# caesar-one/audio-classification-using-a-deep-cnn-combined-with-multi-level-attention

Measured on AMD Instinct MI355X. Metric: 0.96 s clips/sec wave->logits (VGGish+attn), higher is better.
Workload: dtype bf16; 1 GPU; BASELINE config 3: wave->logits forward, 1024 bags x 10 s 16 kHz PCM per GPU = 10240 x 0.96 s clips per step, VGGish + MLA [2,1], random-init portable-seeded weights; f32 front-end/head, bf16 conv+FC; bags_per_gpu=1024, parallelism=dp1 (no collective: independent bags)

## Files before the change

### audio-classification-using-a-deep-cnn-combined-with-multi-level-attention_amd/_lib.py

```python

import ctypes
import os
import re

HERE = os.path.dirname(os.path.abspath(__file__))
LIB_PATH = os.environ.get("MLA_HIP_LIB") or os.path.join(HERE, "libmla_hip.so")
HEADER = os.path.join(os.path.dirname(HERE), "include", "mla_hip.h")

F32, BF16, I16, BF16X3, F64, I32 = 0, 1, 2, 3, 4, 5
E_SHORT = -3

_lib = None


class MlaError(RuntimeError):
    def __init__(self, code, msg):
        super().__init__("libmla_hip error %d: %s" % (code, msg))
        self.code = code


def declared_symbols():
    text = open(HEADER).read()
    text = re.sub(r"/\*.*?\*/", "", text, flags=re.S)
    return sorted(set(re.findall(r"\b(mla_[a-z0-9_]+)\s*\(", text)))
# ... 3 lines not shown
    global _lib
    if _lib is None:
        if not os.path.exists(LIB_PATH):
            raise RuntimeError(
                "%s is missing: build it with `python __graft_entry__.py` (hipcc --offload-arch=gfx950). "
                "There is no fallback path." % LIB_PATH)
        import torch
        L = ctypes.CDLL(LIB_PATH)
        L.mla_last_error.restype = ctypes.c_char_p
        L.mla_logmel_table_floats.restype = ctypes.c_int64
        i64, vp, ci = ctypes.c_int64, ctypes.c_void_p, ctypes.c_int
        L.mla_logmel_counts.argtypes = [i64, ctypes.POINTER(i64), ctypes.POINTER(i64)]
        L.mla_logmel_build_tables.argtypes = [vp]
        L.mla_logmel_reference_tables.argtypes = [vp, vp]
        L.mla_logmel_examples.argtypes = [vp, ci, i64, i64, i64, vp, vp, ci, vp]
        cf = ctypes.c_float
        L.mla_stft_magnitude.argtypes = [vp, i64, vp, vp, i64, i64, i64, vp, vp]
        L.mla_mel_log.argtypes = [vp, vp, i64, i64, i64, cf, vp, vp]
        L.mla_dataset_frames.argtypes = [vp, i64, ci, ci, ci, ci, vp, vp]
        L.mla_postprocess.argtypes = [vp, vp, vp, i64, vp, vp]
        L.mla_mono_mix.argtypes = [vp, ci, i64, ci, vp, vp]
        L.mla_split_bf16x3.argtypes = [vp, i64, i64, i64, vp, i64, i64, ci, vp]
        L.mla_merge_bf16x3.argtypes = [vp, i64, i64, i64, i64, vp, vp]
        L.mla_linear_bf16x3.argtypes = [vp, i64, vp, i64, vp, vp, i64, i64, i64, i64, i64, ci, ci, vp]
        L.mla_conv_repack_weights.argtypes = [vp, i64, i64, vp, ci, vp]
        L.mla_convert_f32.argtypes = [vp, vp, i64, ci, vp]
        L.mla_convert_bf16_to_f32.argtypes = [vp, vp, i64, vp]
        L.mla_vggish_conv1.argtypes = [vp, ci, i64, vp, vp, vp, ci, vp]
        L.mla_vggish_conv.argtypes = [ci, vp, vp, vp, vp, i64, ci, vp]
        L.mla_linear.argtypes = [vp, i64, vp, i64, vp, vp, i64, i64, i64, i64, ci, ci, ci, vp]
# ... 97 lines not shown
```

### audio-classification-using-a-deep-cnn-combined-with-multi-level-attention_amd/csrc/conv.hip

```cpp
#include <cstdlib>
#include <type_traits>

#include "common.h"
#include "mma_core.h"

namespace {

using namespace mma;

constexpr int kThreads = 512, kWaves = 8, kMS = 6;

#ifndef MLA_CONV_STAMPS
#define MLA_CONV_STAMPS 0
#endif
#ifndef MLA_STAMP_TAP
#define MLA_STAMP_TAP 4
#define MLA_STAMP_CHUNK 5
#endif
#if MLA_CONV_STAMPS
__device__ unsigned long long g_conv_stamps[8][2][8];
#define MLA_STAMP(k) do { if (stamp_on) stamps[k] = __builtin_amdgcn_s_memtime(); } while (0)
#if MLA_CONV_STAMPS == 2
#undef MLA_STAMP
#define MLA_STAMP(k) do { } while (0)
// ... 604 lines not shown
    __builtin_amdgcn_wave_barrier();
    __builtin_amdgcn_fence(__ATOMIC_ACQUIRE, "wavefront");
    constexpr int PIECES = 64 * int(sizeof(T)) / 16;
    char* dst = reinterpret_cast<char*>(out + ((size_t(img) * 48 + y0 / 2 + wave) * 32) * 64);
    _Pragma("unroll") for (int it = 0; it < PIECES / 2; ++it) {
        const int piece = it * 64 + lane, p = piece / PIECES, c = piece % PIECES;
        *reinterpret_cast<u32x4*>(dst + size_t(piece) * 16) = *reinterpret_cast<const u32x4*>(stage + p * ROW + c * 16);
    }
    __syncthreads();
    }
}

template <typename TIN>
__global__ __launch_bounds__(256, MLA_CONV1_WAVES) void conv1_patch_kernel(const TIN* __restrict__ x, const float* __restrict__ w,
                                                            const float* __restrict__ bias, bf16_t* __restrict__ out, int n_img) {
    typedef float f32x16 __attribute__((ext_vector_type(16)));
    constexpr int TR = MLA_CONV1_ROWS;
    constexpr int TPC = 96 / TR;
    constexpr int NP = (TR + 2) * 66;
    constexpr int NL = (NP + 255) / 256;
    constexpr int PITCH = 68;
    constexpr int ROW = 64 * 2 + 16;
    __shared__ __attribute__((aligned(16))) uint16_t sX[(TR + 2) * PITCH];
    __shared__ __attribute__((aligned(16))) char sOut[4 * 32 * ROW];
    const int t = threadIdx.x, lane = t & 63, wave = t >> 6, px = lane & 31, h = lane >> 5;
    const int n_tiles = n_img * TPC;

    bf16x8 wa[4][2];
    f32x16 binit[2];
    {
        const int rho = px;
        const int chl = 16 * ((rho >> 2) & 1) + (rho & 3) + 4 * (rho >> 3);
        _Pragma("unroll") for (int pos = 0; pos < 4; ++pos) {
            const int dy = pos >> 1, dx = pos & 1;
            _Pragma("unroll") for (int mt = 0; mt < 2; ++mt) {
                const int ch = mt * 32 + chl;
                uint32_t pk[4];
                _Pragma("unroll") for (int jj = 0; jj < 4; ++jj) {
                    float v[2];
                    _Pragma("unroll") for (int e = 0; e < 2; ++e) {
                        const int k = 8 * h + 2 * jj + e, i = k >> 2, c = k & 3;
                        const int ky = i - dy, kx = c - dx;
                        v[e] = (ky >= 0 && ky < 3 && kx >= 0 && kx < 3) ? w[ch * 9 + ky * 3 + kx] : 0.f;
                    }
                    pk[jj] = pack_bf16x2(v[0], v[1]);
                }
                wa[pos][mt] = __builtin_bit_cast(bf16x8, u32x4{pk[0], pk[1], pk[2], pk[3]});
            }
        }
        _Pragma("unroll") for (int mt = 0; mt < 2; ++mt)
            _Pragma("unroll") for (int reg = 0; reg < 16; ++reg) binit[mt][reg] = bias[mt * 32 + 16 * h + reg];
    }

    float pre[NL];
    auto patch_load = [&](int tile) {
        const int img = tile / TPC, y0 = (tile % TPC) * TR;
        _Pragma("unroll") for (int k = 0; k < NL; ++k) {
            const int p = t + 256 * k, yh = p / 66, xh = p % 66;
            const int gy = y0 + yh - 1, gx = xh - 1;
            const int cy = gy < 0 ? 0 : (gy > 95 ? 95 : gy), cx = gx < 0 ? 0 : (gx > 63 ? 63 : gx);
            const float v = load_elem<TIN>(x + (size_t(img) * 96 + cy) * 64 + cx);
            pre[k] = (p < NP && gy >= 0 && gy < 96 && gx >= 0 && gx < 64) ? v : 0.f;
        }
    };
    auto patch_write = [&]() {
        _Pragma("unroll") for (int k = 0; k < NL; ++k) {
            const int p = t + 256 * k;
// ... 6 lines not shown
        __builtin_amdgcn_s_barrier();
#else
        __syncthreads();
#endif
    };
    int tile = blockIdx.x;
    if (tile < n_tiles) patch_load(tile);
    char* stage = sOut + wave * 32 * ROW;
    for (; tile < n_tiles; tile += gridDim.x) {
        const int img = tile / TPC, y0 = (tile % TPC) * TR;
        patch_write();
        lds_barrier();
        if (tile + int(gridDim.x) < n_tiles) patch_load(tile + int(gridDim.x));
        _Pragma("unroll") for (int rr = 0; rr < TR / 8; ++rr) {
            const int prow = wave * (TR / 8) + rr;
            const uint32_t* r0 = reinterpret_cast<const uint32_t*>(sX + (2 * prow + 2 * h) * PITCH) + px;
            const uint32_t* r1 = reinterpret_cast<const uint32_t*>(sX + (2 * prow + 2 * h + 1) * PITCH) + px;
            const bf16x8 bfrag = __builtin_bit_cast(bf16x8, u32x4{r0[0], r0[1], r1[0], r1[1]});
            _Pragma("unroll") for (int mt = 0; mt < 2; ++mt) {
                f32x16 m = __builtin_amdgcn_mfma_f32_32x32x16_bf16(wa[0][mt], bfrag, binit[mt], 0, 0, 0);
                _Pragma("unroll") for (int pos = 1; pos < 4; ++pos) {
                    const f32x16 a = __builtin_amdgcn_mfma_f32_32x32x16_bf16(wa[pos][mt], bfrag, binit[mt], 0, 0, 0);
                    _Pragma("unroll") for (int reg = 0; reg < 16; ++reg) m[reg] = fmaxf(m[reg], a[reg]);
                }
                uint32_t pk[8];
                _Pragma("unroll") for (int e = 0; e < 8; ++e) pk[e] = pack_bf16x2(fmaxf(m[2 * e], 0.f), fmaxf(m[2 * e + 1], 0.f));
                char* dst = stage + px * ROW + (mt * 32 + 16 * h) * 2;
                *reinterpret_cast<u32x4*>(dst) = u32x4{pk[0], pk[1], pk[2], pk[3]};
                *reinterpret_cast<u32x4*>(dst + 16) = u32x4{pk[4], pk[5], pk[6], pk[7]};
            }
            __builtin_amdgcn_fence(__ATOMIC_RELEASE, "wavefront");
            __builtin_amdgcn_wave_barrier();
            __builtin_amdgcn_fence(__ATOMIC_ACQUIRE, "wavefront");
            char* gdst = reinterpret_cast<char*>(out + ((size_t(img) * 48 + y0 / 2 + prow) * 32) * 64);
            _Pragma("unroll") for (int it = 0; it < 4; ++it) {
                const int piece = it * 64 + lane, p = piece >> 3, c = piece & 7;
#if MLA_CONV_NT_STORE
                __builtin_nontemporal_store(*reinterpret_cast<const u32x4*>(stage + p * ROW + c * 16), reinterpret_cast<u32x4*>(gdst + size_t(piece) * 16));
#else
                *reinterpret_cast<u32x4*>(gdst + size_t(piece) * 16) = *reinterpret_cast<const u32x4*>(stage + p * ROW + c * 16);
#endif
            }
            __builtin_amdgcn_fence(__ATOMIC_RELEASE, "wavefront");
            __builtin_amdgcn_wave_barrier();
            __builtin_amdgcn_fence(__ATOMIC_ACQUIRE, "wavefront");
        }
        lds_barrier();
    }
}

template <typename T>
__global__ void repack_kernel(const float* __restrict__ w, T* __restrict__ out, int cout, int cin) {
    const int64_t total = int64_t(cout) * 9 * cin;
    for (int64_t i = int64_t(blockIdx.x) * blockDim.x + threadIdx.x; i < total; i += int64_t(gridDim.x) * blockDim.x) {
        const int c = int(i % cin);
        const int tap = int((i / cin) % 9);
        const int o = int(i / (int64_t(cin) * 9));
        store_elem<T>(out + i, w[(int64_t(o) * cin + c) * 9 + tap]);
    }
}
// ... 325 lines not shown
```

### audio-classification-using-a-deep-cnn-combined-with-multi-level-attention_amd/csrc/logmel.hip

```cpp
#include <hip/hip_bf16.h>

#include "common.h"
#include "logmel_core.h"
#include "logmel_tables.h"

namespace {

using namespace logmel;

#ifndef MLA_LOGMEL_STAMPS
#define MLA_LOGMEL_STAMPS 0
#endif
#if MLA_LOGMEL_STAMPS
__device__ unsigned long long g_logmel_stamps[256][10];
#endif

constexpr int kPair = 2;
constexpr int kChunk = 16 * kPair;
constexpr int kThreads = 256;
constexpr int kWgPerCu = 2;
constexpr int kXchFloats = 2 * 16 * kXchStride;
constexpr int kWinFloats = 416;
constexpr int kPwPitch = 18;
constexpr int kU = 18;
// ... 102 lines not shown
        _Pragma("unroll") for (int e = 0; e < 4; ++e) {
            _Pragma("unroll") for (int s = 0; s < 4; ++s) {
                if (t < count[s]) {
                    acc_a[s] += w[first[s] / 4 + t][e] * a[first[s] / 4 + t][e];
                    acc_b[s] += w[first[s] / 4 + t][e] * b[first[s] / 4 + t][e];
                }
            }
        }
    }
    _Pragma("unroll") for (int s = 0; s < 4; ++s) {
        oa[s] = __builtin_amdgcn_logf(acc_a[s] + 0.01f) * 0.69314718055994530942f;
        ob[s] = __builtin_amdgcn_logf(acc_b[s] + 0.01f) * 0.69314718055994530942f;
    }
}

template <typename OutT>
__device__ __forceinline__ void store_piece(OutT* dst, f32x4 v) {
    if constexpr (sizeof(OutT) == 4) {
        *reinterpret_cast<f32x4*>(dst) = v;
    } else {
        const __hip_bfloat16 b0 = __float2bfloat16(v.x), b1 = __float2bfloat16(v.y), b2 = __float2bfloat16(v.z), b3 = __float2bfloat16(v.w);
        auto bits = [](const __hip_bfloat16& h) { return uint32_t(*reinterpret_cast<const uint16_t*>(&h)); };
        *reinterpret_cast<u32x2*>(dst) = u32x2{bits(b0) | (bits(b1) << 16), bits(b2) | (bits(b3) << 16)};
    }
}

template <typename InT, typename OutT, bool VEC, bool WAVE>
__device__ __forceinline__ void pair_step(const LaneConsts& c, int j, Samples<InT>& smp, const InT* next_frame, float* xa, float* xb,
                                          const float* s_win, const float* melw, const float* pw, OutT* dst) {
    float ra[16], ia[16], rb[16], ib[16];
    {
        _Pragma("unroll") for (int n1 = 0; n1 < kN1; ++n1) {
            const f32x2 w = *reinterpret_cast<const f32x2*>(s_win + 32 * n1 + 2 * j);
            const f32x2 a = smp.pair(n1), b = smp.pair(n1 + 5);
            ra[n1] = a.x * w.x; ia[n1] = a.y * w.y;
            rb[n1] = b.x * w.x; ib[n1] = b.y * w.y;
        }
    }
    if (next_frame) smp.template fetch<VEC>(next_frame, j);
    phase1_fft(c, j, ra, ia, xa);
    group_sync<WAVE>();
    phase1_fft(c, j, rb, ib, xb);
    group_sync<WAVE>();
    read_row(xa + 2 * (j * kXchStride), ra, ia);
// ... 5 lines not shown
    }
    __builtin_amdgcn_sched_barrier(0);
    group_sync<WAVE>();
    phase2_fft(ra, ia);
    split_frame<WAVE>(j, ra, ia, xa, pwl);
    phase2_fft(rb, ib);
    split_frame<WAVE>(j, rb, ib, xb, pwl);
    group_sync<WAVE>();
    float oa[4], ob[4];
    mel_pair(c, xa, xb, melw, oa, ob);
    _Pragma("unroll") for (int s = 0; s < 4; ++s) { xa[256 + band_of(j, s)] = oa[s]; xb[256 + band_of(j, s)] = ob[s]; }
    group_sync<WAVE>();
    {
        const f32x4 va = *reinterpret_cast<const f32x4*>(xa + 256 + 4 * j);
        const f32x4 vb = *reinterpret_cast<const f32x4*>(xb + 256 + 4 * j);
        store_piece<OutT>(dst + 4 * j, va);
        store_piece<OutT>(dst + kBands + 4 * j, vb);
    }
    group_sync<WAVE>();
}

template <typename InT, typename OutT, bool VEC, bool WAVE>
__global__ __launch_bounds__(kThreads, kWgPerCu) void logmel_kernel(const InT* __restrict__ pcm, ChunkMap map,
                                                              int64_t n_chunks, const float* __restrict__ tab,
                                                              OutT* __restrict__ out) {
    extern __shared__ __attribute__((aligned(16))) float smem[];
    float* s_xch = smem;
    float* s_mel = s_xch + kChunk * kXchFloats;
    float* s_pw = s_mel + 16 * kMelRow;
    float* s_win = s_pw + 16 * kPwPitch;

    const int t = threadIdx.x, g = t >> 4, j = t & 15;
// ... 12 lines not shown
    Samples<InT> smp;
    int64_t chunk = blockIdx.x, sample0, row0;
    if (chunk < n_chunks) {
        map.locate(chunk, sample0, row0);
        smp.template fetch<VEC>(pcm + sample0 + (kPair * g) * kHop, j);
    }
    for (; chunk < n_chunks; chunk += gridDim.x) {
        map.locate(chunk, sample0, row0);
        const int64_t next = chunk + gridDim.x;
        const InT* next_frame = nullptr;
        if (next < n_chunks) {
            int64_t ns, nr;
            map.locate(next, ns, nr);
            next_frame = pcm + ns + (kPair * g) * kHop;
        }
        pair_step<InT, OutT, VEC, WAVE>(c, j, smp, next_frame, xa, xb, s_win, melw, pw, out + (row0 + kPair * g) * kBands);
    }
}

constexpr int kThreadsDyn = 512;
constexpr int kItemFrames = 4 * kPair;
constexpr int kLdsFloatsDyn = (kThreadsDyn / 16) * kPair * kXchFloats + 16 * kMelRow + 16 * kPwPitch + kWinFloats + 4;
constexpr int kLdsBytesDyn = kLdsFloatsDyn * 4;
static_assert(kLdsBytesDyn <= 160 * 1024 && kChunk % kItemFrames == 0, "dynamic kernel: LDS / item size");

template <typename InT, typename OutT, bool VEC>
__global__ __launch_bounds__(kThreadsDyn, 1) void logmel_dyn_kernel(const InT* __restrict__ pcm, ChunkMap map, int64_t n_items,
                                                                    const float* __restrict__ tab, OutT* __restrict__ out) {
    extern __shared__ __attribute__((aligned(16))) float smem[];
    float* s_xch = smem;
    float* s_mel = s_xch + (kThreadsDyn / 16) * kPair * kXchFloats;
// ... 39 lines not shown
    if (cur < hi) {
        locate_item(cur, sample, row);
        smp.template fetch<VEC>(pcm + sample + lane_frame * kHop, j);
    }
#if MLA_LOGMEL_STAMPS
    const unsigned long long stamp0 = __builtin_amdgcn_s_memrealtime();
#endif
    while (cur < hi) {
        const int nxt = pull();
        int64_t nsample = 0, nrow = 0;
        const InT* next_frame = nullptr;
        if (nxt < hi) {
            locate_item(nxt, nsample, nrow);
            next_frame = pcm + nsample + lane_frame * kHop;
        }
        pair_step<InT, OutT, VEC, true>(c, j, smp, next_frame, xa, xb, s_win, melw, pw, out + (row + lane_frame) * kBands);
        cur = nxt;
        row = nrow;
    }
#if MLA_LOGMEL_STAMPS
    if (lane == 0 && blockIdx.x < 256) {
        if (t == 0) { g_logmel_stamps[blockIdx.x][0] = stamp_entry; g_logmel_stamps[blockIdx.x][9] = stamp0; }
        g_logmel_stamps[blockIdx.x][1 + (t >> 6)] = __builtin_amdgcn_s_memrealtime();
    }
#endif
}

template <typename InT, typename OutT>
int launch(const void* pcm, int64_t n_wave, int64_t wave_stride, int64_t examples, const float* tables,
           void* out, bool wave_sync, bool static_wave, hipStream_t stream) {
    const int64_t n_chunks = n_wave * examples * (kExFrames / kChunk);
    if (n_chunks == 0) return MLA_OK;
    const bool vec = mla::aligned(pcm, 2 * sizeof(InT)) && (wave_stride % 2 == 0);
    int dev = 0, cus = 256;
    if (hipGetDevice(&dev) == hipSuccess) hipDeviceGetAttribute(&cus, hipDeviceAttributeMultiprocessorCount, dev);
    const int64_t grid = n_chunks < kWgPerCu * int64_t(cus) ? n_chunks : kWgPerCu * int64_t(cus);
    ChunkMap map{wave_stride, int(examples * (kExFrames / kChunk))};
    auto go = [&](auto kern) -> int {
        MLA_HIP_OK(hipFuncSetAttribute(reinterpret_cast<const void*>(kern),
                                       hipFuncAttributeMaxDynamicSharedMemorySize, kLdsBytes));
// ... 70 lines not shown
    MLA_REQUIRE(pcm && tables && out, MLA_E_ARG, "null pcm/tables/out");
    MLA_REQUIRE(mla::aligned(out, 16) && mla::aligned(tables, 4), MLA_E_ARG, "out must be 16-byte aligned");
    MLA_REQUIRE(pcm_dtype == MLA_F32 || pcm_dtype == MLA_I16, MLA_E_DTYPE, "pcm_dtype %d", pcm_dtype);
    MLA_REQUIRE(out_dtype == MLA_F32 || out_dtype == MLA_BF16, MLA_E_DTYPE, "out_dtype %d", out_dtype);
    MLA_REQUIRE(mla::aligned(pcm, pcm_dtype == MLA_F32 ? 4 : 2), MLA_E_ARG, "pcm misaligned for its dtype");
    const char* env = getenv("MLA_LOGMEL_SYNC");
    const bool wave_sync = !(env && env[0] == 'b'), static_wave = env && env[0] == 's';
    hipStream_t s = static_cast<hipStream_t>(stream);
    if (pcm_dtype == MLA_F32) {
        return out_dtype == MLA_F32 ? launch<float, float>(pcm, n_wave, wave_stride, examples, tables, out, wave_sync, static_wave, s)
                                    : launch<float, __hip_bfloat16>(pcm, n_wave, wave_stride, examples, tables, out, wave_sync, static_wave, s);
    }
    return out_dtype == MLA_F32 ? launch<int16_t, float>(pcm, n_wave, wave_stride, examples, tables, out, wave_sync, static_wave, s)
                                : launch<int16_t, __hip_bfloat16>(pcm, n_wave, wave_stride, examples, tables, out, wave_sync, static_wave, s);
}
```

### audio-classification-using-a-deep-cnn-combined-with-multi-level-attention_amd/model.py

```python

from typing import Dict, List, Union

import torch
from torch import nn

from . import differentiable, mla_train, ops, resnet
from .params import *
from .torchvggish.vggish import Linear, VGGish


class BatchNorm1d(nn.Module):

    def __init__(self, num_features):
        super().__init__()
        self.num_features, self.eps, self.momentum = num_features, 1e-5, 0.1
        self.weight = nn.Parameter(torch.ones(num_features))
        self.bias = nn.Parameter(torch.zeros(num_features))
        self.register_buffer("running_mean", torch.zeros(num_features))
        self.register_buffer("running_var", torch.ones(num_features))
        self.register_buffer("num_batches_tracked", torch.tensor(0, dtype=torch.long))

    def forward(self, x):
        raise RuntimeError("BatchNorm1d is executed by the fused HIP head of its parent module")

# ... 56 lines not shown
    def forward(self, x):
        x_proc = self.input(x)
        features = self.cnn(x_proc)
        out = self.mla(features.reshape(-1, T, self.emb_input_size))
        return out

    def _waveforms_only_vggish(self):
        if self.cnn_type != "vggish":
            raise NotImplementedError("the waveform paths feed VGGish log-mel examples; cnn_type 'resnet' takes 224 x 224 "
                                      "spectrogram images (dataset.py:175-178 of the reference) through forward()")

    def forward_waveforms(self, pcm):
        self._waveforms_only_vggish()
        from . import frontend
        dtype = torch.bfloat16 if self.cnn.precision == "bf16" else torch.float32
        ex = frontend.waveforms_to_examples(pcm, out_dtype=dtype)
        assert ex.shape[0] == pcm.shape[0] * T, "each waveform must yield exactly T examples"
        features = self.cnn(ex)
        return self.mla(features.reshape(-1, T, self.emb_input_size))

    def stream_waveforms(self, host_batches):
        self._waveforms_only_vggish()
        dev = next(self.parameters()).device
        cur = torch.cuda.current_stream(dev)
        copy = torch.cuda.Stream(device=dev)
        it = iter(host_batches)

        def upload(host):
            assert host.is_pinned(), "stream_waveforms overlaps asynchronous copies: the host tensors must be pinned"
            with torch.cuda.stream(copy):
# ... 204 lines not shown
```

### audio-classification-using-a-deep-cnn-combined-with-multi-level-attention_amd/ops.py

```python

import ctypes

import torch

from . import _lib

DT = {torch.float32: _lib.F32, torch.bfloat16: _lib.BF16, torch.int16: _lib.I16}
BN_EPS = 1e-5

profile = None
_ws = {}


_event_pool = []


def reserve_events(n):
    while len(_event_pool) < n:
        e = torch.cuda.Event(enable_timing=True)
        e.record()
        _event_pool.append(e)
    torch.cuda.synchronize()


# ... 75 lines not shown

def to_f32(x):
    _chk(x, torch.bfloat16)
    out = torch.empty(x.shape, dtype=torch.float32, device=x.device)
    _lib.check(_lib.lib().mla_convert_bf16_to_f32(_p(x), _p(out), x.numel(), _lib.stream_ptr()))
    return out


def conv1(x, w, b, dtype, split=False):
    _chk(x); _chk(w, torch.float32); _chk(b, torch.float32)
    n = x.shape[0]
    assert tuple(x.shape[1:]) == (96, 64) and tuple(w.shape) == (64, 1, 3, 3)
    out = torch.empty((n, 48, 32, 128 if split else 64), dtype=dtype, device=x.device)
    _lib.check(_timed("conv1", _lib.lib().mla_vggish_conv1, _p(x), DT[x.dtype], n, _p(w), _p(b), _p(out),
                      _lib.BF16X3 if split else DT[dtype], _lib.stream_ptr()))
    return out


CONV_SHAPES = {2: ((48, 32, 64), (24, 16, 128)), 3: ((24, 16, 128), (24, 16, 256)), 4: ((24, 16, 256), (12, 8, 256)),
               5: ((12, 8, 256), (12, 8, 512)), 6: ((12, 8, 512), (6, 4, 512))}


def conv(layer, x, w_packed, b, split=False):
    _chk(x); _chk(w_packed, x.dtype); _chk(b, torch.float32)
    shp_in, shp_out = CONV_SHAPES[layer]
    ka, kw, ko = (2, 3, 2) if split else (1, 1, 1)
    assert tuple(x.shape[1:]) == shp_in[:2] + (ka * shp_in[2],), (x.shape, shp_in)
    assert tuple(w_packed.shape) == (shp_out[2], 9, kw * shp_in[2])
    n = x.shape[0]
    out = torch.empty((n,) + shp_out[:2] + (ko * shp_out[2],), dtype=x.dtype, device=x.device)
# ... 680 lines not shown
```

### audio-classification-using-a-deep-cnn-combined-with-multi-level-attention_amd/torchvggish/vggish.py

```python

import math

import numpy as np
import torch
import torch.nn as nn

from . import vggish_input, vggish_params
from .. import ops

_DTYPES = {"f32": torch.float32, "bf16": torch.bfloat16, "bf16x3": torch.bfloat16}


class Conv3x3(nn.Module):

    def __init__(self, in_channels, out_channels):
        super().__init__()
        self.in_channels, self.out_channels = in_channels, out_channels
        self.weight = nn.Parameter(torch.empty(out_channels, in_channels, 3, 3))
        self.bias = nn.Parameter(torch.empty(out_channels))
        nn.init.kaiming_uniform_(self.weight, a=math.sqrt(5))
        bound = 1.0 / math.sqrt(in_channels * 9)
        nn.init.uniform_(self.bias, -bound, bound)

    def forward(self, x):
# ... 13 lines not shown
    pass


class _Cache:

    def __init__(self):
        self.key, self.val = None, None

    def get(self, params, dtype, make):
        key = (dtype,) + tuple((p.data_ptr(), p._version) for p in params)
        if key != self.key:
            self.key, self.val = key, make()
        return self.val


class VGGFeatures(nn.Sequential):

    precision = "f32"

    def __init__(self, *layers):
        super().__init__(*layers)
        self._cache = _Cache()
        convs = [m for m in self if isinstance(m, Conv3x3)]
        assert [(c.in_channels, c.out_channels) for c in convs] == [(1, 64), (64, 128), (128, 256), (256, 256), (256, 512), (512, 512)]
        self._convs = convs

    def forward_nhwc(self, x, dtype):
        x = x.detach().reshape(-1, 96, 64)
        if x.dtype not in (torch.float32, torch.bfloat16):
            x = x.float()
        x = x.contiguous()
        convs = self._convs
        if self.precision == "bf16x3":
            packed = self._cache.get([c.weight for c in convs[1:]], "bf16x3",
                                     lambda: [ops.split_conv_weight(c.weight.detach().contiguous()) for c in convs[1:]])
            h = ops.conv1(x.float(), convs[0].weight.detach().contiguous(), convs[0].bias.detach(), torch.bfloat16, split=True)
            for layer, (c, w) in enumerate(zip(convs[1:], packed), start=2):
                h = ops.conv(layer, h, w, c.bias.detach(), split=True)
            return h
        packed = self._cache.get([c.weight for c in convs[1:]], dtype,
                                 lambda: [ops.repack_conv_weight(c.weight.detach().contiguous(), dtype) for c in convs[1:]])
        h = ops.conv1(x, convs[0].weight.detach().contiguous(), convs[0].bias.detach(), dtype)
        for layer, (c, w) in enumerate(zip(convs[1:], packed), start=2):
            h = ops.conv(layer, h, w, c.bias.detach())
        return h

    def forward(self, x):
        from .. import differentiable as D
        if D.wants_grad(self):
            params = [t for i in (0, 3, 6, 8, 11, 13) for t in (self[i].weight, self[i].bias)]
            return D.FeaturesFn.apply(self, D.grad_precision(self.precision), x, *params).permute(0, 3, 1, 2)
        return self.forward_nhwc(x, _DTYPES[self.precision]).permute(0, 3, 1, 2)


class Linear(nn.Module):

    def __init__(self, in_features, out_features):
        super().__init__()
        self.in_features, self.out_features = in_features, out_features
        self.weight = nn.Parameter(torch.empty(out_features, in_features))
        self.bias = nn.Parameter(torch.empty(out_features))
        nn.init.kaiming_uniform_(self.weight, a=math.sqrt(5))
        bound = 1.0 / math.sqrt(in_features)
# ... 134 lines not shown
```

### include/mla_hip.h

```cpp
#ifndef MLA_HIP_H
#define MLA_HIP_H

#include <stdint.h>

#ifdef __cplusplus
extern "C" {
#endif

#define MLA_OK            0
#define MLA_E_ARG        -1
#define MLA_E_SHAPE      -2
#define MLA_E_SHORT      -3
#define MLA_E_LAUNCH     -4
#define MLA_E_DTYPE      -5

#define MLA_F32   0
#define MLA_BF16  1
#define MLA_I16   2
#define MLA_F64   4
#define MLA_I32   5
#define MLA_BF16X3 3

typedef void* mla_stream_t;

// ... 24 lines not shown
                    float* out, mla_stream_t stream);


int mla_conv_repack_weights(const float* w_oihw, int64_t cout, int64_t cin, void* out, int dtype,
                            mla_stream_t stream);
int mla_convert_f32(const float* in, void* out, int64_t n, int dtype, mla_stream_t stream);
int mla_convert_bf16_to_f32(const void* in, float* out, int64_t n, mla_stream_t stream);
int mla_split_bf16x3(const float* in, int64_t rows, int64_t cols, int64_t ld_in, void* out, int64_t ld_out, int64_t seg,
                     int copies, mla_stream_t stream);
int mla_merge_bf16x3(const void* in, int64_t rows, int64_t cols, int64_t ld_in, int64_t seg, float* out, mla_stream_t stream);
int mla_linear_bf16x3(const void* a, int64_t lda, const void* w, int64_t ldw, const float* bias, void* out, int64_t ldo,
                      int64_t M, int64_t N, int64_t K, int64_t seg, int out_dtype, int relu, mla_stream_t stream);

int mla_vggish_conv1(const void* x, int x_dtype, int64_t n, const float* w, const float* bias, void* out,
                     int dtype, mla_stream_t stream);

int mla_vggish_conv(int layer, const void* in, const void* w_repacked, const float* bias, void* out,
                    int64_t n, int dtype, mla_stream_t stream);

int mla_linear(const void* a, int64_t lda, const void* w, int64_t ldw, const float* bias, void* out,
               int64_t ldo, int64_t M, int64_t N, int64_t K, int dtype, int out_dtype, int relu,
               mla_stream_t stream);
int mla_linear_ksplit(const void* a, int64_t lda, const void* w, int64_t ldw, const float* bias, void* out, int64_t ldo,
                      int64_t M, int64_t N, int64_t K, int dtype, int out_dtype, int relu, int splits, float* workspace,
                      int64_t workspace_floats, mla_stream_t stream);
int mla_linear_splitk(const float* a, int64_t lda, const float* w, int64_t ldw, const float* bias, float* out,
                      int64_t ldo, int64_t M, int64_t N, int64_t K, int relu, int splits, float* workspace,
                      int64_t workspace_floats, mla_stream_t stream);
int mla_linear_narrow(const float* a, int64_t lda, const float* w, int64_t ldw, const float* bias, float* out,
                      int64_t ldo, int64_t M, int64_t N, int64_t K, mla_stream_t stream);
// ... 162 lines not shown
```

Measured before the change: 858,700 clips/s.

## Fuse log-mel front end with conv1+pool into one persistent kernel

```diff
diff --git a/audio-classification-using-a-deep-cnn-combined-with-multi-level-attention_amd/_lib.py b/audio-classification-using-a-deep-cnn-combined-with-multi-level-attention_amd/_lib.py
--- a/audio-classification-using-a-deep-cnn-combined-with-multi-level-attention_amd/_lib.py
+++ b/audio-classification-using-a-deep-cnn-combined-with-multi-level-attention_amd/_lib.py
@@ -41,6 +41,7 @@
         L.mla_logmel_build_tables.argtypes = [vp]
         L.mla_logmel_reference_tables.argtypes = [vp, vp]
         L.mla_logmel_examples.argtypes = [vp, ci, i64, i64, i64, vp, vp, ci, vp]
+        L.mla_logmel_conv1.argtypes = [vp, ci, i64, i64, i64, vp, vp, vp, vp, vp]
         cf = ctypes.c_float
         L.mla_stft_magnitude.argtypes = [vp, i64, vp, vp, i64, i64, i64, vp, vp]
         L.mla_mel_log.argtypes = [vp, vp, i64, i64, i64, cf, vp, vp]
diff --git a/audio-classification-using-a-deep-cnn-combined-with-multi-level-attention_amd/csrc/conv.hip b/audio-classification-using-a-deep-cnn-combined-with-multi-level-attention_amd/csrc/conv.hip
--- a/audio-classification-using-a-deep-cnn-combined-with-multi-level-attention_amd/csrc/conv.hip
+++ b/audio-classification-using-a-deep-cnn-combined-with-multi-level-attention_amd/csrc/conv.hip
@@ -2,6 +2,7 @@
 #include <type_traits>
 
 #include "common.h"
+#include "conv1_core.h"
 #include "mma_core.h"
 
 namespace {
@@ -642,13 +643,13 @@
 template <typename TIN>
 __global__ __launch_bounds__(256, MLA_CONV1_WAVES) void conv1_patch_kernel(const TIN* __restrict__ x, const float* __restrict__ w,
                                                             const float* __restrict__ bias, bf16_t* __restrict__ out, int n_img) {
-    typedef float f32x16 __attribute__((ext_vector_type(16)));
+    using conv1::f32x16;
     constexpr int TR = MLA_CONV1_ROWS;
     constexpr int TPC = 96 / TR;
     constexpr int NP = (TR + 2) * 66;
     constexpr int NL = (NP + 255) / 256;
-    constexpr int PITCH = 68;
-    constexpr int ROW = 64 * 2 + 16;
+    constexpr int PITCH = conv1::kPitch;
+    constexpr int ROW = conv1::kStageRow;
     __shared__ __attribute__((aligned(16))) uint16_t sX[(TR + 2) * PITCH];
     __shared__ __attribute__((aligned(16))) char sOut[4 * 32 * ROW];
     const int t = threadIdx.x, lane = t & 63, wave = t >> 6, px = lane & 31, h = lane >> 5;
@@ -656,29 +657,9 @@
 
     bf16x8 wa[4][2];
     f32x16 binit[2];
-    {
-        const int rho = px;
-        const int chl = 16 * ((rho >> 2) & 1) + (rho & 3) + 4 * (rho >> 3);
-        _Pragma("unroll") for (int pos = 0; pos < 4; ++pos) {
-            const int dy = pos >> 1, dx = pos & 1;
-            _Pragma("unroll") for (int mt = 0; mt < 2; ++mt) {
-                const int ch = mt * 32 + chl;
-                uint32_t pk[4];
-                _Pragma("unroll") for (int jj = 0; jj < 4; ++jj) {
-                    float v[2];
-                    _Pragma("unroll") for (int e = 0; e < 2; ++e) {
-                        const int k = 8 * h + 2 * jj + e, i = k >> 2, c = k & 3;
-                        const int ky = i - dy, kx = c - dx;
-                        v[e] = (ky >= 0 && ky < 3 && kx >= 0 && kx < 3) ? w[ch * 9 + ky * 3 + kx] : 0.f;
-                    }
-                    pk[jj] = pack_bf16x2(v[0], v[1]);
-                }
-                wa[pos][mt] = __builtin_bit_cast(bf16x8, u32x4{pk[0], pk[1], pk[2], pk[3]});
-            }
-        }
-        _Pragma("unroll") for (int mt = 0; mt < 2; ++mt)
-            _Pragma("unroll") for (int reg = 0; reg < 16; ++reg) binit[mt][reg] = bias[mt * 32 + 16 * h + reg];
-    }
+    _Pragma("unroll") for (int pos = 0; pos < 4; ++pos)
+        _Pragma("unroll") for (int mt = 0; mt < 2; ++mt) wa[pos][mt] = conv1::weight_frag(w, pos, mt, lane);
+    _Pragma("unroll") for (int mt = 0; mt < 2; ++mt) binit[mt] = conv1::bias_frag(bias, mt, lane);
 
     float pre[NL];
     auto patch_load = [&](int tile) {
@@ -715,36 +696,8 @@
         if (tile + int(gridDim.x) < n_tiles) patch_load(tile + int(gridDim.x));
         _Pragma("unroll") for (int rr = 0; rr < TR / 8; ++rr) {
             const int prow = wave * (TR / 8) + rr;
-            const uint32_t* r0 = reinterpret_cast<const uint32_t*>(sX + (2 * prow + 2 * h) * PITCH) + px;
-            const uint32_t* r1 = reinterpret_cast<const uint32_t*>(sX + (2 * prow + 2 * h + 1) * PITCH) + px;
-            const bf16x8 bfrag = __builtin_bit_cast(bf16x8, u32x4{r0[0], r0[1], r1[0], r1[1]});
-            _Pragma("unroll") for (int mt = 0; mt < 2; ++mt) {
-                f32x16 m = __builtin_amdgcn_mfma_f32_32x32x16_bf16(wa[0][mt], bfrag, binit[mt], 0, 0, 0);
-                _Pragma("unroll") for (int pos = 1; pos < 4; ++pos) {
-                    const f32x16 a = __builtin_amdgcn_mfma_f32_32x32x16_bf16(wa[pos][mt], bfrag, binit[mt], 0, 0, 0);
-                    _Pragma("unroll") for (int reg = 0; reg < 16; ++reg) m[reg] = fmaxf(m[reg], a[reg]);
-                }
-                uint32_t pk[8];
-                _Pragma("unroll") for (int e = 0; e < 8; ++e) pk[e] = pack_bf16x2(fmaxf(m[2 * e], 0.f), fmaxf(m[2 * e + 1], 0.f));
-                char* dst = stage + px * ROW + (mt * 32 + 16 * h) * 2;
-                *reinterpret_cast<u32x4*>(dst) = u32x4{pk[0], pk[1], pk[2], pk[3]};
-                *reinterpret_cast<u32x4*>(dst + 16) = u32x4{pk[4], pk[5], pk[6], pk[7]};
-            }
-            __builtin_amdgcn_fence(__ATOMIC_RELEASE, "wavefront");
-            __builtin_amdgcn_wave_barrier();
-            __builtin_amdgcn_fence(__ATOMIC_ACQUIRE, "wavefront");
             char* gdst = reinterpret_cast<char*>(out + ((size_t(img) * 48 + y0 / 2 + prow) * 32) * 64);
-            _Pragma("unroll") for (int it = 0; it < 4; ++it) {
-                const int piece = it * 64 + lane, p = piece >> 3, c = piece & 7;
-#if MLA_CONV_NT_STORE
-                __builtin_nontemporal_store(*reinterpret_cast<const u32x4*>(stage + p * ROW + c * 16), reinterpret_cast<u32x4*>(gdst + size_t(piece) * 16));
-#else
-                *reinterpret_cast<u32x4*>(gdst + size_t(piece) * 16) = *reinterpret_cast<const u32x4*>(stage + p * ROW + c * 16);
-#endif
-            }
-            __builtin_amdgcn_fence(__ATOMIC_RELEASE, "wavefront");
-            __builtin_amdgcn_wave_barrier();
-            __builtin_amdgcn_fence(__ATOMIC_ACQUIRE, "wavefront");
+            conv1::pooled_row(sX + (2 * prow) * PITCH, wa, binit, stage, gdst, lane);
         }
         lds_barrier();
     }
diff --git a/audio-classification-using-a-deep-cnn-combined-with-multi-level-attention_amd/csrc/conv1_core.h b/audio-classification-using-a-deep-cnn-combined-with-multi-level-attention_amd/csrc/conv1_core.h
--- /dev/null
+++ b/audio-classification-using-a-deep-cnn-combined-with-multi-level-attention_amd/csrc/conv1_core.h
@@ -0,0 +1,79 @@
+#ifndef MLA_CONV1_CORE_H
+#define MLA_CONV1_CORE_H
+
+#include "mma_core.h"
+
+#ifndef MLA_CONV_NT_STORE
+#define MLA_CONV_NT_STORE 1
+#endif
+
+namespace conv1 {
+
+using namespace mma;
+
+typedef float f32x16 __attribute__((ext_vector_type(16)));
+
+constexpr int kPitch = 68;
+constexpr int kStageRow = 64 * 2 + 16;
+constexpr int kStageBytes = 32 * kStageRow;
+
+__device__ __forceinline__ bf16x8 weight_frag(const float* __restrict__ w, int pos, int mt, int lane) {
+    const int rho = lane & 31, h = lane >> 5;
+    const int chl = 16 * ((rho >> 2) & 1) + (rho & 3) + 4 * (rho >> 3);
+    const int dy = pos >> 1, dx = pos & 1;
+    const int ch = mt * 32 + chl;
+    uint32_t pk[4];
+    _Pragma("unroll") for (int jj = 0; jj < 4; ++jj) {
+        float v[2];
+        _Pragma("unroll") for (int e = 0; e < 2; ++e) {
+            const int k = 8 * h + 2 * jj + e, i = k >> 2, c = k & 3;
+            const int ky = i - dy, kx = c - dx;
+            v[e] = (ky >= 0 && ky < 3 && kx >= 0 && kx < 3) ? w[ch * 9 + ky * 3 + kx] : 0.f;
+        }
+        pk[jj] = pack_bf16x2(v[0], v[1]);
+    }
+    return __builtin_bit_cast(bf16x8, u32x4{pk[0], pk[1], pk[2], pk[3]});
+}
+
+__device__ __forceinline__ f32x16 bias_frag(const float* bias, int mt, int lane) {
+    f32x16 b;
+    _Pragma("unroll") for (int reg = 0; reg < 16; ++reg) b[reg] = bias[mt * 32 + 16 * (lane >> 5) + reg];
+    return b;
+}
+
+__device__ __forceinline__ void pooled_row(const uint16_t* rows, const bf16x8 (&wa)[4][2], const f32x16 (&binit)[2], char* stage,
+                                           char* gdst, int lane) {
+    const int px = lane & 31, h = lane >> 5;
+    const uint32_t* r0 = reinterpret_cast<const uint32_t*>(rows + (2 * h) * kPitch) + px;
+    const uint32_t* r1 = reinterpret_cast<const uint32_t*>(rows + (2 * h + 1) * kPitch) + px;
+    const bf16x8 bfrag = __builtin_bit_cast(bf16x8, u32x4{r0[0], r0[1], r1[0], r1[1]});
+    _Pragma("unroll") for (int mt = 0; mt < 2; ++mt) {
+        f32x16 m = __builtin_amdgcn_mfma_f32_32x32x16_bf16(wa[0][mt], bfrag, binit[mt], 0, 0, 0);
+        _Pragma("unroll") for (int pos = 1; pos < 4; ++pos) {
+            const f32x16 a = __builtin_amdgcn_mfma_f32_32x32x16_bf16(wa[pos][mt], bfrag, binit[mt], 0, 0, 0);
+            _Pragma("unroll") for (int reg = 0; reg < 16; ++reg) m[reg] = fmaxf(m[reg], a[reg]);
+        }
+        uint32_t pk[8];
+        _Pragma("unroll") for (int e = 0; e < 8; ++e) pk[e] = pack_bf16x2(fmaxf(m[2 * e], 0.f), fmaxf(m[2 * e + 1], 0.f));
+        char* dst = stage + px * kStageRow + (mt * 32 + 16 * h) * 2;
+        *reinterpret_cast<u32x4*>(dst) = u32x4{pk[0], pk[1], pk[2], pk[3]};
+        *reinterpret_cast<u32x4*>(dst + 16) = u32x4{pk[4], pk[5], pk[6], pk[7]};
+    }
+    __builtin_amdgcn_fence(__ATOMIC_RELEASE, "wavefront");
+    __builtin_amdgcn_wave_barrier();
+    __builtin_amdgcn_fence(__ATOMIC_ACQUIRE, "wavefront");
+    _Pragma("unroll") for (int it = 0; it < 4; ++it) {
+        const int piece = it * 64 + lane, p = piece >> 3, c = piece & 7;
+#if MLA_CONV_NT_STORE
+        __builtin_nontemporal_store(*reinterpret_cast<const u32x4*>(stage + p * kStageRow + c * 16), reinterpret_cast<u32x4*>(gdst + size_t(piece) * 16));
+#else
+        *reinterpret_cast<u32x4*>(gdst + size_t(piece) * 16) = *reinterpret_cast<const u32x4*>(stage + p * kStageRow + c * 16);
+#endif
+    }
+    __builtin_amdgcn_fence(__ATOMIC_RELEASE, "wavefront");
+    __builtin_amdgcn_wave_barrier();
+    __builtin_amdgcn_fence(__ATOMIC_ACQUIRE, "wavefront");
+}
+
+}
+#endif
diff --git a/audio-classification-using-a-deep-cnn-combined-with-multi-level-attention_amd/csrc/logmel.hip b/audio-classification-using-a-deep-cnn-combined-with-multi-level-attention_amd/csrc/logmel.hip
--- a/audio-classification-using-a-deep-cnn-combined-with-multi-level-attention_amd/csrc/logmel.hip
+++ b/audio-classification-using-a-deep-cnn-combined-with-multi-level-attention_amd/csrc/logmel.hip
@@ -1,6 +1,7 @@
 #include <hip/hip_bf16.h>
 
 #include "common.h"
+#include "conv1_core.h"
 #include "logmel_core.h"
 #include "logmel_tables.h"
 
@@ -140,20 +141,48 @@
     }
 }
 
+__device__ __forceinline__ u32x2 pack_piece(f32x4 v) {
+    const __hip_bfloat16 b0 = __float2bfloat16(v.x), b1 = __float2bfloat16(v.y), b2 = __float2bfloat16(v.z), b3 = __float2bfloat16(v.w);
+    auto bits = [](const __hip_bfloat16& h) { return uint32_t(*reinterpret_cast<const uint16_t*>(&h)); };
+    return u32x2{bits(b0) | (bits(b1) << 16), bits(b2) | (bits(b3) << 16)};
+}
+
 template <typename OutT>
 __device__ __forceinline__ void store_piece(OutT* dst, f32x4 v) {
     if constexpr (sizeof(OutT) == 4) {
         *reinterpret_cast<f32x4*>(dst) = v;
     } else {
-        const __hip_bfloat16 b0 = __float2bfloat16(v.x), b1 = __float2bfloat16(v.y), b2 = __float2bfloat16(v.z), b3 = __float2bfloat16(v.w);
-        auto bits = [](const __hip_bfloat16& h) { return uint32_t(*reinterpret_cast<const uint16_t*>(&h)); };
-        *reinterpret_cast<u32x2*>(dst) = u32x2{bits(b0) | (bits(b1) << 16), bits(b2) | (bits(b3) << 16)};
-    }
-}
-
-template <typename InT, typename OutT, bool VEC, bool WAVE>
+        *reinterpret_cast<u32x2*>(dst) = pack_piece(v);
+    }
+}
+
+template <typename OutT>
+struct RowsToGlobal {
+    OutT* dst;
+    __device__ __forceinline__ void operator()(int j, f32x4 va, f32x4 vb) const {
+        store_piece<OutT>(dst + 4 * j, va);
+        store_piece<OutT>(dst + kBands + 4 * j, vb);
+    }
+};
+struct RowsToStaged {
+    uint16_t* row;
+    __device__ __forceinline__ void one(uint16_t* r, int j, f32x4 v) const {
+        const u32x2 p = pack_piece(v);
+        r[4 * j + 1] = uint16_t(p.x);
+        *reinterpret_cast<uint32_t*>(r + 4 * j + 2) = (p.x >> 16) | (p.y << 16);
+        r[4 * j + 4] = uint16_t(p.y >> 16);
+        if (j == 0) r[0] = 0;
+        if (j == 15) r[65] = 0;
+    }
+    __device__ __forceinline__ void operator()(int j, f32x4 va, f32x4 vb) const {
+        one(row, j, va);
+        one(row + conv1::kPitch, j, vb);
+    }
+};
+
+template <typename InT, bool VEC, bool WAVE, typename Sink>
 __device__ __forceinline__ void pair_step(const LaneConsts& c, int j, Samples<InT>& smp, const InT* next_frame, float* xa, float* xb,
-                                          const float* s_win, const float* melw, const float* pw, OutT* dst) {
+                                          const float* s_win, const float* melw, const float* pw, const Sink& sink) {
     float ra[16], ia[16], rb[16], ib[16];
     {
         _Pragma("unroll") for (int n1 = 0; n1 < kN1; ++n1) {
@@ -189,8 +218,8 @@
     {
         const f32x4 va = *reinterpret_cast<const f32x4*>(xa + 256 + 4 * j);
         const f32x4 vb = *reinterpret_cast<const f32x4*>(xb + 256 + 4 * j);
-        store_piece<OutT>(dst + 4 * j, va);
-        store_piece<OutT>(dst + kBands + 4 * j, vb);
+        group_sync<WAVE>();
+        sink(j, va, vb);
     }
     group_sync<WAVE>();
 }
@@ -233,7 +262,7 @@
             map.locate(next, ns, nr);
             next_frame = pcm + ns + (kPair * g) * kHop;
         }
-        pair_step<InT, OutT, VEC, WAVE>(c, j, smp, next_frame, xa, xb, s_win, melw, pw, out + (row0 + kPair * g) * kBands);
+        pair_step<InT, VEC, WAVE>(c, j, smp, next_frame, xa, xb, s_win, melw, pw, RowsToGlobal<OutT>{out + (row0 + kPair * g) * kBands});
     }
 }
 
@@ -303,7 +332,7 @@
             locate_item(nxt, nsample, nrow);
             next_frame = pcm + nsample + lane_frame * kHop;
         }
-        pair_step<InT, OutT, VEC, true>(c, j, smp, next_frame, xa, xb, s_win, melw, pw, out + (row + lane_frame) * kBands);
+        pair_step<InT, VEC, true>(c, j, smp, next_frame, xa, xb, s_win, melw, pw, RowsToGlobal<OutT>{out + (row + lane_frame) * kBands});
         cur = nxt;
         row = nrow;
     }
@@ -313,6 +342,133 @@
         g_logmel_stamps[blockIdx.x][1 + (t >> 6)] = __builtin_amdgcn_s_memrealtime();
     }
 #endif
+}
+
+constexpr int kClipItems = kExFrames / kItemFrames;
+constexpr int kFusedWaBytes = 8 * 64 * 16;
+constexpr int kLdsBytesFused = kLdsBytesDyn + kFusedWaBytes + 64 * 4;
+constexpr int kStagedDwords = conv1::kPitch / 2;
+static_assert(kLdsBytesDyn % 16 == 0 && kLdsBytesFused <= 160 * 1024, "fused kernel: LDS");
+static_assert(12 * conv1::kPitch * 2 <= kXchFloats * 4 && conv1::kStageBytes <= 2 * kXchFloats * 4 && kItemFrames * kXchFloats >= 3 * kXchFloats,
+              "staged rows in the wave's first exchange buffer, output stage in the next two");
+static_assert(kThreadsDyn / 64 == 8, "one wave per (position, channel tile) builds the weight fragments");
+
+template <typename InT, bool VEC>
+__global__ __launch_bounds__(kThreadsDyn, 1) void logmel_conv1_kernel(const InT* __restrict__ pcm, int64_t wave_stride, int examples,
+                                                                      int n_clips, const float* __restrict__ tab,
+                                                                      const float* __restrict__ w, const float* __restrict__ bias,
+                                                                      mma::bf16_t* __restrict__ out) {
+    extern __shared__ __attribute__((aligned(16))) float smem[];
+    float* s_xch = smem;
+    float* s_mel = s_xch + (kThreadsDyn / 16) * kPair * kXchFloats;
+    float* s_pw = s_mel + 16 * kMelRow;
+    float* s_win = s_pw + 16 * kPwPitch;
+    int* s_next = reinterpret_cast<int*>(s_win + kWinFloats);
+    mma::u32x4* s_wa = reinterpret_cast<mma::u32x4*>(smem + kLdsFloatsDyn);
+    float* s_bias = smem + kLdsFloatsDyn + kFusedWaBytes / 4;
+
+    const int t = threadIdx.x, g = t >> 4, gl = g & 3, j = t & 15, lane = t & 63, wv = __builtin_amdgcn_readfirstlane(t >> 6);
+    float* xa = s_xch + (kPair * g) * kXchFloats;
+    float* xb = xa + kXchFloats;
+    char* wregion = reinterpret_cast<char*>(s_xch + (kItemFrames * wv) * kXchFloats);
+    uint16_t* sX = reinterpret_cast<uint16_t*>(wregion);
+    uint32_t* sX32 = reinterpret_cast<uint32_t*>(wregion);
+    char* stage = wregion + kXchFloats * 4;
+
+    LaneConsts c;
+    load_consts(c, tab, j);
+    for (int i = t; i < 16 * kMelRow; i += kThreadsDyn) s_mel[i] = tab[kTabMelW + i];
+    for (int i = t; i < 16 * kPwRow; i += kThreadsDyn) s_pw[(i >> 4) * kPwPitch + (i & 15)] = tab[kTabPw + i];
+    for (int i = t; i < kWinFloats; i += kThreadsDyn) s_win[i] = tab[kTabWindow + i];
+    s_wa[t] = __builtin_bit_cast(mma::u32x4, conv1::weight_frag(w, wv >> 1, wv & 1, lane));
+    if (t < 64) s_bias[t] = bias[t];
+    const int lo = int(int64_t(n_clips) * int64_t(blockIdx.x) / int64_t(gridDim.x)), hi = int(int64_t(n_clips) * (int64_t(blockIdx.x) + 1) / int64_t(gridDim.x));
+    if (t == 0) *s_next = lo;
+    const float* melw = s_mel + kMelRow * j;
+    const float* pw = s_pw + kPwPitch * j;
+    __syncthreads();
+
+    auto pull = [&]() {
+        int v = 0;
+        if (lane == 0) v = atomicAdd(s_next, 1);
+        return __builtin_amdgcn_readfirstlane(v);
+    };
+    const int lane_frame = kPair * gl;
+    auto item_frame = [&](int clip, int item) {
+        const int wf = clip / examples, e = clip - wf * examples;
+        return pcm + int64_t(wf) * wave_stride + (int64_t(e) * kExFrames + item * kItemFrames + lane_frame) * kHop;
+    };
+    auto wave_fence = [&]() {
+        __builtin_amdgcn_fence(__ATOMIC_RELEASE, "wavefront");
+        __builtin_amdgcn_wave_barrier();
+        __builtin_amdgcn_fence(__ATOMIC_ACQUIRE, "wavefront");
+    };
+    Samples<InT> smp;
+    int clip = pull(), item = 0;
+    if (clip < hi) smp.template fetch<VEC>(item_frame(clip, 0), j);
+    uint32_t* parked = reinterpret_cast<uint32_t*>(wregion) + 3 * kXchFloats;
+    auto park_slot = [](int d) { return (d / 28) * kXchFloats + 2 * kXchStride * (9 + (d % 28) / 4) + 32 + d % 4; };
+    const int second = 64 + lane < 3 * kStagedDwords ? 64 + lane : 3 * kStagedDwords - 1;
+    auto conv_item = [&](int clip, int item) {
+        {
+            const uint32_t k0 = parked[park_slot(lane)], k1 = parked[park_slot(second)];
+            sX32[lane] = item == 0 ? 0u : k0;
+            if (lane < 3 * kStagedDwords - 64) sX32[64 + lane] = item == 0 ? 0u : k1;
+        }
+        if (lane < kStagedDwords) sX32[11 * kStagedDwords + lane] = 0u;
+        wave_fence();
+        {
+            mma::bf16x8 wa[4][2];
+            conv1::f32x16 binit[2];
+            _Pragma("unroll") for (int pos = 0; pos < 4; ++pos)
+                _Pragma("unroll") for (int mt = 0; mt < 2; ++mt) wa[pos][mt] = __builtin_bit_cast(mma::bf16x8, s_wa[(pos * 2 + mt) * 64 + lane]);
+            _Pragma("unroll") for (int mt = 0; mt < 2; ++mt) binit[mt] = conv1::bias_frag(s_bias, mt, lane);
+            auto row = [&](int q) {
+                char* gdst = reinterpret_cast<char*>(out + ((size_t(clip) * 48 + size_t(4 * item - 1 + q)) * 32) * 64);
+                conv1::pooled_row(sX + (2 * q) * conv1::kPitch, wa, binit, stage, gdst, lane);
+            };
+            if (item == kClipItems - 1) row(4);
+            row(item == 0 ? 1 : 0);
+            row(1);
+            row(2);
+            row(3);
+        }
+        {
+            const uint32_t k0 = sX32[8 * kStagedDwords + lane], k1 = sX32[8 * kStagedDwords + second];
+            parked[park_slot(lane)] = k0;
+            parked[park_slot(second)] = k1;
+        }
+        wave_fence();
+    };
+    while (clip < hi) {
+        int nclip = clip, nitem = item + 1;
+        if (nitem == kClipItems) { nclip = pull(); nitem = 0; }
+        const InT* next_frame = nclip < hi ? item_frame(nclip, nitem) : nullptr;
+        pair_step<InT, VEC, true>(c, j, smp, next_frame, xa, xb, s_win, melw, pw, RowsToStaged{sX + (3 + lane_frame) * conv1::kPitch});
+        conv_item(clip, item);
+        clip = nclip;
+        item = nitem;
+    }
+}
+
+template <typename InT>
+int launch_fused(const void* pcm, int64_t n_wave, int64_t wave_stride, int64_t examples, const float* tables, const float* w,
+                 const float* bias, void* out, hipStream_t stream) {
+    const int64_t n_clips = n_wave * examples;
+    if (n_clips == 0) return MLA_OK;
+    MLA_REQUIRE(n_clips <= 0x7fffffff / kClipItems, MLA_E_SHAPE, "too many clips for one launch (%lld)", (long long)n_clips);
+    const bool vec = mla::aligned(pcm, 2 * sizeof(InT)) && (wave_stride % 2 == 0);
+    int dev = 0, cus = 256;
+    if (hipGetDevice(&dev) == hipSuccess) hipDeviceGetAttribute(&cus, hipDeviceAttributeMultiprocessorCount, dev);
+    const int64_t wgs = n_clips < cus ? n_clips : cus;
+    auto go = [&](auto kern) -> int {
+        MLA_HIP_OK(hipFuncSetAttribute(reinterpret_cast<const void*>(kern), hipFuncAttributeMaxDynamicSharedMemorySize, kLdsBytesFused));
+        hipLaunchKernelGGL(kern, dim3(unsigned(wgs)), dim3(kThreadsDyn), kLdsBytesFused, stream, static_cast<const InT*>(pcm), wave_stride,
+                           int(examples), int(n_clips), tables, w, bias, static_cast<mma::bf16_t*>(out));
+        MLA_LAUNCH_OK("logmel_conv1_kernel");
+        return MLA_OK;
+    };
+    return vec ? go(logmel_conv1_kernel<InT, true>) : go(logmel_conv1_kernel<InT, false>);
 }
 
 template <typename InT, typename OutT>
@@ -413,3 +569,21 @@
     return out_dtype == MLA_F32 ? launch<int16_t, float>(pcm, n_wave, wave_stride, examples, tables, out, wave_sync, static_wave, s)
                                 : launch<int16_t, __hip_bfloat16>(pcm, n_wave, wave_stride, examples, tables, out, wave_sync, static_wave, s);
 }
+
+extern "C" int mla_logmel_conv1(const void* pcm, int pcm_dtype, int64_t n_wave, int64_t n_samples, int64_t wave_stride,
+                                const float* tables, const float* w, const float* bias, void* out, mla_stream_t stream) {
+    MLA_REQUIRE(n_wave >= 0 && wave_stride >= n_samples, MLA_E_ARG, "bad n_wave %lld / stride %lld < n_samples %lld",
+                (long long)n_wave, (long long)wave_stride, (long long)n_samples);
+    int64_t frames = 0, examples = 0;
+    const int rc = mla_logmel_counts(n_samples, &frames, &examples);
+    if (rc != MLA_OK) return rc;
+    if (n_wave == 0 || examples == 0) return MLA_OK;
+    MLA_REQUIRE(pcm && tables && w && bias && out, MLA_E_ARG, "null pcm/tables/w/bias/out");
+    MLA_REQUIRE(mla::aligned(out, 16) && mla::aligned(tables, 4) && mla::aligned(w, 4) && mla::aligned(bias, 4), MLA_E_ARG,
+                "out must be 16-byte aligned");
+    MLA_REQUIRE(pcm_dtype == MLA_F32 || pcm_dtype == MLA_I16, MLA_E_DTYPE, "pcm_dtype %d", pcm_dtype);
+    MLA_REQUIRE(mla::aligned(pcm, pcm_dtype == MLA_F32 ? 4 : 2), MLA_E_ARG, "pcm misaligned for its dtype");
+    hipStream_t s = static_cast<hipStream_t>(stream);
+    return pcm_dtype == MLA_F32 ? launch_fused<float>(pcm, n_wave, wave_stride, examples, tables, w, bias, out, s)
+                                : launch_fused<int16_t>(pcm, n_wave, wave_stride, examples, tables, w, bias, out, s);
+}
diff --git a/audio-classification-using-a-deep-cnn-combined-with-multi-level-attention_amd/model.py b/audio-classification-using-a-deep-cnn-combined-with-multi-level-attention_amd/model.py
--- a/audio-classification-using-a-deep-cnn-combined-with-multi-level-attention_amd/model.py
+++ b/audio-classification-using-a-deep-cnn-combined-with-multi-level-attention_amd/model.py
@@ -6,7 +6,7 @@
 
 from . import differentiable, mla_train, ops, resnet
 from .params import *
-from .torchvggish.vggish import Linear, VGGish
+from .torchvggish.vggish import Linear, PcmInput, VGGish
 
 
 class BatchNorm1d(nn.Module):
@@ -94,6 +94,11 @@
         self._waveforms_only_vggish()
         from . import frontend
         dtype = torch.bfloat16 if self.cnn.precision == "bf16" else torch.float32
+        feats = self.cnn.cnn_model[0] if self.just_bottlenecks else self.cnn.cnn_model.features
+        if ops.FUSED_FRONT and dtype == torch.bfloat16 and not differentiable.wants_grad(feats):
+            assert pcm.dim() == 2 and frontend.counts(pcm.shape[1])[1] == T, "each waveform must yield exactly T examples"
+            features = self.cnn(PcmInput(pcm))
+            return self.mla(features.reshape(-1, T, self.emb_input_size))
         ex = frontend.waveforms_to_examples(pcm, out_dtype=dtype)
         assert ex.shape[0] == pcm.shape[0] * T, "each waveform must yield exactly T examples"
         features = self.cnn(ex)
diff --git a/audio-classification-using-a-deep-cnn-combined-with-multi-level-attention_amd/ops.py b/audio-classification-using-a-deep-cnn-combined-with-multi-level-attention_amd/ops.py
--- a/audio-classification-using-a-deep-cnn-combined-with-multi-level-attention_amd/ops.py
+++ b/audio-classification-using-a-deep-cnn-combined-with-multi-level-attention_amd/ops.py
@@ -1,5 +1,6 @@
 
 import ctypes
+import os
 
 import torch
 
@@ -113,6 +114,25 @@
     out = torch.empty((n, 48, 32, 128 if split else 64), dtype=dtype, device=x.device)
     _lib.check(_timed("conv1", _lib.lib().mla_vggish_conv1, _p(x), DT[x.dtype], n, _p(w), _p(b), _p(out),
                       _lib.BF16X3 if split else DT[dtype], _lib.stream_ptr()))
+    return out
+
+
+FUSED_FRONT = os.environ.get("MLA_FUSED_FRONT", "1") != "0"
+
+
+def logmel_conv1(pcm, w, b):
+    from . import frontend
+    assert pcm.dim() == 2 and pcm.is_cuda and pcm.stride(1) == 1 and pcm.dtype in (torch.float32, torch.int16)
+    _chk(w, torch.float32); _chk(b, torch.float32)
+    assert tuple(w.shape) == (64, 1, 3, 3)
+    n_wave, n_samples = pcm.shape
+    _, n_ex = frontend.counts(n_samples)
+    out = torch.empty((n_wave * n_ex, 48, 32, 64), dtype=torch.bfloat16, device=pcm.device)
+    if n_wave * n_ex == 0:
+        return out
+    tab = frontend.device_tables(pcm.device)
+    _lib.check(_timed("logmel", _lib.lib().mla_logmel_conv1, _p(pcm), DT[pcm.dtype], n_wave, n_samples,
+                      pcm.stride(0) if n_wave > 1 else n_samples, _p(tab), _p(w), _p(b), _p(out), _lib.stream_ptr()))
     return out
 
 
diff --git a/audio-classification-using-a-deep-cnn-combined-with-multi-level-attention_amd/torchvggish/vggish.py b/audio-classification-using-a-deep-cnn-combined-with-multi-level-attention_amd/torchvggish/vggish.py
--- a/audio-classification-using-a-deep-cnn-combined-with-multi-level-attention_amd/torchvggish/vggish.py
+++ b/audio-classification-using-a-deep-cnn-combined-with-multi-level-attention_amd/torchvggish/vggish.py
@@ -51,6 +51,12 @@
         return self.val
 
 
+class PcmInput:
+
+    def __init__(self, pcm):
+        self.pcm = pcm
+
+
 class VGGFeatures(nn.Sequential):
 
     precision = "f32"
@@ -63,6 +69,15 @@
         self._convs = convs
 
     def forward_nhwc(self, x, dtype):
+        convs = self._convs
+        if isinstance(x, PcmInput):
+            assert dtype == torch.bfloat16 and self.precision == "bf16", "the fused front is the bf16 inference path"
+            packed = self._cache.get([c.weight for c in convs[1:]], dtype,
+                                     lambda: [ops.repack_conv_weight(c.weight.detach().contiguous(), dtype) for c in convs[1:]])
+            h = ops.logmel_conv1(x.pcm, convs[0].weight.detach().contiguous(), convs[0].bias.detach())
+            for layer, (c, w) in enumerate(zip(convs[1:], packed), start=2):
+                h = ops.conv(layer, h, w, c.bias.detach())
+            return h
         x = x.detach().reshape(-1, 96, 64)
         if x.dtype not in (torch.float32, torch.bfloat16):
             x = x.float()
@@ -84,6 +99,8 @@
 
     def forward(self, x):
         from .. import differentiable as D
+        if isinstance(x, PcmInput):
+            return self.forward_nhwc(x, _DTYPES[self.precision]).permute(0, 3, 1, 2)
         if D.wants_grad(self):
             params = [t for i in (0, 3, 6, 8, 11, 13) for t in (self[i].weight, self[i].bias)]
             return D.FeaturesFn.apply(self, D.grad_precision(self.precision), x, *params).permute(0, 3, 1, 2)
diff --git a/include/mla_hip.h b/include/mla_hip.h
--- a/include/mla_hip.h
+++ b/include/mla_hip.h
@@ -62,6 +62,9 @@
 
 int mla_vggish_conv1(const void* x, int x_dtype, int64_t n, const float* w, const float* bias, void* out,
                      int dtype, mla_stream_t stream);
+
+int mla_logmel_conv1(const void* pcm, int pcm_dtype, int64_t n_wave, int64_t n_samples, int64_t wave_stride,
+                     const float* tables, const float* w, const float* bias, void* out, mla_stream_t stream);
 
 int mla_vggish_conv(int layer, const void* in, const void* w_repacked, const float* bias, void* out,
                     int64_t n, int dtype, mla_stream_t stream);
```

Result: faster. 868,200 clips/s, median of 6 (+1.1%).
